# littlemesie/recommend-tf2.0

Hardware: NVIDIA B200
Metric: DLRM train samples/sec (higher is better)
Workload: dtype f32

## Files before the change

### include/rtf_b200.h

```cpp
#ifndef RTF_B200_H
#define RTF_B200_H

#include <stddef.h>
#include <stdint.h>

#ifdef __cplusplus
extern "C" {
#endif

#define RTF_MAX_FIELDS 64

#define RTF_E_ARG (-1)
#define RTF_E_ALIGN (-2)
#define RTF_E_RANGE (-3)
#define RTF_E_WORKSPACE (-4)

enum { RTF_POOL_NONE = 0, RTF_POOL_SUM = 1, RTF_POOL_MEAN = 2,
       RTF_POOL_SKIP_INVALID = 0x100 };
enum { RTF_OPT_NONE = 0, RTF_OPT_SGD = 1, RTF_OPT_ADAGRAD = 2, RTF_OPT_ADAM = 3 };

typedef struct rtf_opt {
  int32_t kind;
  float lr;
  float beta1;
// ... 176 lines not shown
int rtf_layernorm_workspace(int64_t rows, int C, size_t* bytes);
int rtf_layernorm_fwd(const float* d_x, int64_t rows, int C, const float* d_gamma,
                      const float* d_beta, float eps, float* d_y, float* d_mean, float* d_rstd,
                      void* stream);
int rtf_layernorm_bwd(const float* d_dy, const float* d_x, const float* d_mean, const float* d_rstd,
                      const float* d_gamma, int64_t rows, int C, float* d_dx, float* d_dgamma,
                      float* d_dbeta, void* d_ws, size_t ws_bytes, void* stream);

int rtf_dense_gemm_nn_workspace(int M, int N, int K, int batch, size_t* bytes);
int rtf_dense_gemm_nt_workspace(int M, int N, int K, int batch, size_t* bytes);
int rtf_dense_gemm_tn_workspace(int M, int N, int K, int batch, size_t* bytes);
int rtf_dense_gemm_nn(const float* d_a, int64_t lda, int64_t stride_a, const float* d_b, int64_t ldb,
                      int64_t stride_b, const float* d_bias, int relu, float* d_out, int64_t ldd,
                      int64_t stride_d, int M, int N, int K, int batch, void* d_ws, size_t ws_bytes,
                      void* stream);
int rtf_dense_gemm_nt(const float* d_a, int64_t lda, int64_t stride_a, const float* d_b, int64_t ldb,
                      int64_t stride_b, const float* d_bias, int relu, float* d_out, int64_t ldd,
                      int64_t stride_d, int M, int N, int K, int batch, void* d_ws, size_t ws_bytes,
                      void* stream);
int rtf_dense_gemm_tn(const float* d_a, int64_t lda, int64_t stride_a, const float* d_b, int64_t ldb,
                      int64_t stride_b, const float* d_bias, int relu, float* d_out, int64_t ldd,
                      int64_t stride_d, int M, int N, int K, int batch, void* d_ws, size_t ws_bytes,
                      void* stream);

int rtf_autoint_layer_supported(int F, int dm, int H, int hs);
int rtf_autoint_layer_workspace(int64_t B, int dm, int HS, size_t* bytes);
int rtf_autoint_layer_fwd(const float* d_x, int64_t B, int F, int dm, const float* d_wq,
                          const float* d_wk, const float* d_wv, const float* d_w0, int H, int hs,
                          int act, float scale, float* d_out, void* stream);
int rtf_autoint_layer_bwd(const float* d_x, int64_t B, int F, int dm, const float* d_wq,
                          const float* d_wk, const float* d_wv, const float* d_w0, int H, int hs,
                          int act, float scale, const float* d_out, const float* d_gout,
                          float* d_gx, float* d_gw, void* d_ws, size_t ws_bytes, void* stream);

int rtf_sasrec_score_fwd(const float* d_info, int64_t info_sb, const float* d_pos_tab,
                         int64_t pos_rows, const float* d_neg_tab, int64_t neg_rows,
                         const void* d_pos_ids, const void* d_neg_ids, int ids_i64, int64_t neg_sb,
                         int64_t B, int NEG, int D, float* d_logits, float* d_loss_rows,
                         int32_t* d_err, void* stream);
int rtf_sasrec_score_bwd(const float* d_info, int64_t info_sb, const float* d_pos_tab,
                         int64_t pos_rows, const float* d_neg_tab, int64_t neg_rows,
                         const void* d_pos_ids, const void* d_neg_ids, int ids_i64, int64_t neg_sb,
                         int64_t B, int NEG, int D, const float* d_logits, const float* d_gloss,
                         const float* d_glogits, float* d_ginfo, float* d_gemb, void* stream);

int rtf_topk_ip_workspace(int64_t B, int64_t N, int D, int k, size_t* bytes);
// ... 20 lines not shown
```

### recommend-tf2.0_b200/_lib.py

```python
from __future__ import annotations

import ctypes as C
import os
import subprocess
import sys

_HERE = os.path.dirname(os.path.abspath(__file__))
LIB_PATH = os.path.join(_HERE, "librtf_b200.so")
CSRC_DIR = os.path.join(_HERE, "csrc")
HEADER_PATH = os.path.join(os.path.dirname(_HERE), "include", "rtf_b200.h")

POOL_NONE, POOL_SUM, POOL_MEAN = 0, 1, 2
OPT_NONE, OPT_SGD, OPT_ADAGRAD, OPT_ADAM = 0, 1, 2, 3
SEG_CHUNK = 64
MAX_FIELDS = 64


class RtfError(RuntimeError):
    pass


class rtf_opt(C.Structure):
    _fields_ = [("kind", C.c_int32), ("lr", C.c_float), ("beta1", C.c_float),
                ("beta2", C.c_float), ("eps", C.c_float), ("l2", C.c_float),
# ... 50 lines not shown
    "rtf_sasrec_score_bwd": [_p, _i64, _p, _i64, _p, _i64, _p, _p, _int, _i64, _i64, _int, _int, _p, _p, _p,
                             _p, _p, _p],
    "rtf_topk_ip_workspace": [_i64, _i64, _int, _int, C.POINTER(C.c_size_t)],
    "rtf_topk_ip": [_p, _i64, _i64, _p, _i64, _i64, _int, _int, _p, _p, _p, _p, C.c_size_t, _p],
    "rtf_peer_pull_rows": [_p, _p, _i64, _int, C.c_uint64, _p, _int, _int, _p, _int, _i64, _i64, _i64, _p,
                           _i64, _p, _p],
    "rtf_ssm_gather": [_p, _p, _p, _p, _i64, _int, _int, _p, _p, _p, _p],
    "rtf_ssm_logits_fwd": [_p, _i64, _p, _i64, _p, _p, _p, _p, _p, _p, _i64, _i64, _int, _int, _int, _p, _p,
                           _p, _p],
    "rtf_ssm_logits_bwd": [_p, _i64, _p, _i64, _p, _p, _p, _p, _p, _p, _i64, _i64, _int, _int, _int, _p, _p,
                           _p, _p, _i64, _p],
    "rtf_ssm_true_gx": [_p, _p, _p, _i64, _i64, _int, _p, _i64, _p],
    "rtf_dense_adam": [_p, _p, _p, _p, _i64, C.POINTER(rtf_opt), _p],
    "rtf_rows_apply_dense": [_p, _p, _p, _p, _p, _i64, _int, C.POINTER(rtf_opt), _p],
    "rtf_dense_gemm_nn_workspace": [_int, _int, _int, _int, C.POINTER(C.c_size_t)],
    "rtf_dense_gemm_nt_workspace": [_int, _int, _int, _int, C.POINTER(C.c_size_t)],
    "rtf_dense_gemm_tn_workspace": [_int, _int, _int, _int, C.POINTER(C.c_size_t)],
    "rtf_dense_gemm_nn": [_p, _i64, _i64, _p, _i64, _i64, _p, _int, _p, _i64, _i64, _int, _int, _int,
                          _int, _p, C.c_size_t, _p],
    "rtf_dense_gemm_nt": [_p, _i64, _i64, _p, _i64, _i64, _p, _int, _p, _i64, _i64, _int, _int, _int,
                          _int, _p, C.c_size_t, _p],
    "rtf_dense_gemm_tn": [_p, _i64, _i64, _p, _i64, _i64, _p, _int, _p, _i64, _i64, _int, _int, _int,
                          _int, _p, C.c_size_t, _p],
    "rtf_fm_layer_workspace": [_i64, _int, C.POINTER(C.c_size_t)],
    "rtf_fm_layer_fwd": [_p, _i64, _p, _int, _p, _i64, _int, _int, _i64, _int, _int, _p, _p, _p],
    "rtf_fm_layer_bwd": [_p, _i64, _p, _int, _p, _i64, _int, _int, _i64, _int, _int, _p, _p,
                         _i64, _p, _p, _i64, _p, _p],
    "rtf_fm_gather_fwd": [_p, _p, _int, _int, _int, _p, _int, _p, _i64, _p, _int, _i64, _i64,
                          _i64, _p, _p, _p, _p, _p],
    "rtf_fm_gather_bwd": [_p, _p, _int, _int, _int, _p, _int, _p, _i64, _p, _int, _i64, _i64,
                          _i64, _p, _p, _p, _p, _p, _p, _p],
    "rtf_attn_fwd": [_p, _i64, _i64, _p, _i64, _i64, _p, _i64, _i64, _p, _i64, _p, _i64, _int,
                     _int, _int, _int, _int, _int, C.c_float, _p, _i64, _i64, _p, _p, _p],
    "rtf_attn_bwd": [_p, _i64, _i64, _p, _i64, _i64, _p, _i64, _i64, _p, _i64, _p, _i64, _int,
                     _int, _int, _int, _int, _int, C.c_float, _p, _i64, _i64, _p, _p, _p, _i64,
                     _i64, _p, _p, _i64, _i64, _p, _i64, _i64, _p, _i64, _i64, _p],
    "rtf_din_attn_fwd": [_p, _i64, _p, _i64, _p, _i64, _p, _i64, _p, _p, _int, _i64, _int, _int,
                         _p, _i64, _p],
    "rtf_din_attn_bwd": [_p, _i64, _p, _i64, _p, _i64, _p, _i64, _p, _p, _int, _i64, _int, _int,
                         _p, _i64, _p, _i64, _p, _i64, _p, _i64, _p, _p],
    "rtf_log_uniform_workspace": [_int, C.POINTER(C.c_size_t)],
    "rtf_log_uniform_sample": [C.c_uint64, _int, _i64, _p, _p, _p, _p],
    "rtf_log_uniform_sample_dseed": [_p, _int, _i64, _p, _p, _p, _p],
    "rtf_log_uniform_expected": [_p, _i64, _i64, _p, _p, _p],
    "rtf_sampled_softmax_workspace": [_int, _int, C.POINTER(C.c_size_t)],
    "rtf_sampled_softmax_fwd": [_p, _i64, _p, _p, _p, _p, _p, _p, _i64, _i64, _int, _int, _int,
# ... 61 lines not shown
```

### recommend-tf2.0_b200/core.py

```python
from __future__ import annotations

import math
import os
from typing import Callable, Optional, Sequence

import torch
import torch.nn.functional as F


class Layer(torch.nn.Module):

    def __init__(self, name: Optional[str] = None, **kwargs):
        super().__init__()
        self._built = False
        self._name = name

    def build(self, input_shape):
        pass

    def call(self, inputs, **kwargs):
        raise NotImplementedError

    def forward(self, inputs, *args, **kwargs):
        if not self._built:
# ... 76 lines not shown
             lambda x: torch.softmax(x, -1)}
    if act not in table:
        raise ValueError(f"Unknown activation function: {act}")
    return table[act]


class Dense(Layer):

    def __init__(self, units: int, activation=None, use_bias: bool = True,
                 kernel_regularizer=None, **kwargs):
        super().__init__(**kwargs)
        self.units, self.use_bias, self.kernel_regularizer = units, use_bias, kernel_regularizer
        self.activation = get_activation(activation)
        self._act_name = activation if isinstance(activation, str) else None
        if isinstance(activation, torch.nn.Module):
            self.activation_module = activation

    def build(self, input_shape):
        self.kernel = self.add_weight("kernel", (input_shape[-1], self.units), "glorot_uniform",
                                      self.kernel_regularizer)
        self.bias = self.add_weight("bias", (self.units,), "zeros") if self.use_bias else None

    def call(self, x, **kwargs):
        if self.bias is not None and x.dim() >= 2 and x.is_cuda:
            relu = self._act_name == "relu"
            lead = x.shape[:-1]
            x2 = x.reshape(-1, x.shape[-1]) if x.dim() > 2 else x
            y = _DenseFn.apply(x2, self.kernel, self.bias, relu)
            if x.dim() > 2:
                y = y.reshape(*lead, self.units)
            return y if (relu or self.activation is None) else self.activation(y)
        y = torch.matmul(x, self.kernel)
        if self.bias is not None:
            y = y + self.bias
        return self.activation(y) if self.activation is not None else y


DENSE_GEMM = os.environ.get("RTF_DENSE_GEMM", "bf16x6")


def set_dense_gemm(kind: str) -> None:
    global DENSE_GEMM
    if kind not in ("bf16x6", "library"):
        raise ValueError(kind)
    DENSE_GEMM = kind

# ... 2 lines not shown
    if DENSE_GEMM != "bf16x6":
        return False
    for m in mats:
        if not (m.is_cuda and m.dtype == torch.float32 and m.dim() == 2 and m.is_contiguous()
                and m.shape[0] % 4 == 0 and m.shape[1] % 4 == 0 and m.data_ptr() % 16 == 0):
            return False
    return True


def dense_gemm(kind: str, a: torch.Tensor, b: torch.Tensor, bias=None, relu: bool = False,
               splits: int = 1) -> torch.Tensor:
    import ctypes as C
    from . import _lib as L
    lib = L.lib()
    if kind == "nn":
        (M, K), N = a.shape, b.shape[1]
    elif kind == "nt":
        (M, K), N = a.shape, b.shape[0]
    elif kind == "tn":
        (K, M), N = a.shape, b.shape[1]
    else:
        raise ValueError(kind)
    fn = getattr(lib, f"rtf_dense_gemm_{kind}")
    wsq = getattr(lib, f"rtf_dense_gemm_{kind}_workspace")
    lda, ldb = a.stride(0), b.stride(0)
    sa = sb = sd = 0
    batch = 1
    if kind == "tn" and splits > 1:
        if K % splits or (K // splits) % 4:
            raise ValueError("splits must divide K into multiples of 4")
        batch, K = splits, K // splits
        sa, sb, sd = K * lda, K * ldb, M * N
    out = torch.empty((batch, M, N) if batch > 1 else (M, N), dtype=torch.float32, device=a.device)
    key = (kind, M, N, K, batch)
    if key not in _GEMM_WS_BYTES:
        nb = C.c_size_t(0)
        L.check(wsq(M, N, K, batch, C.byref(nb)), f"rtf_dense_gemm_{kind}_workspace")
        _GEMM_WS_BYTES[key] = max(nb.value, 16)
    ws = _scratch(_GEMM_WS_BYTES[key], a.device)
    rc = fn(a.data_ptr(), lda, sa, b.data_ptr(), ldb, sb, None if bias is None else bias.data_ptr(),
            int(relu), out.data_ptr(), N, sd, M, N, K, batch, ws.data_ptr(), ws.numel(),
            L.current_stream_ptr())
    L.check(rc, f"rtf_dense_gemm_{kind}")
    return out.sum(0) if batch > 1 else out


_GEMM_WS_BYTES: dict = {}
_SCRATCH: dict = {}


def _scratch(nbytes: int, device) -> torch.Tensor:
    key = (device.index, torch._C._cuda_getCurrentRawStream(device.index if device.index is not None
                                                            else torch._C._cuda_getDevice()))
    buf = _SCRATCH.get(key)
    if buf is None or buf.numel() < nbytes:
        buf = _SCRATCH[key] = torch.empty(max(nbytes, 1 << 20), dtype=torch.uint8, device=device)
    return buf


def _wgrad_splits(B: int, kin: int, n: int, clusters: int = 74) -> int:
    tiles = ((kin + 255) // 256) * ((n + 127) // 128)
    best, best_eff = 1, 0.0
    s = 1
    while s <= 64 and B % s == 0 and (B // s) % 4 == 0 and B // s >= 512:
        waves = tiles * s / clusters
        eff = waves / -(-tiles * s // clusters)
        if eff > best_eff + 0.02:
# ... 14 lines not shown

def _relu_bwd_bias_grad(gy: torch.Tensor, y):
    B, N = gy.shape
    if gy.is_cuda and N % 4 == 0 and B > 0:
        import ctypes as C
        from . import _lib as L
        gy = gy.contiguous()
        key = ("relu_bwd", B, N)
        if key not in _GEMM_WS_BYTES:
            nb = C.c_size_t(0)
            L.check(L.lib().rtf_relu_bwd_colsum_workspace(B, N, C.byref(nb)), "rtf_relu_bwd_colsum_workspace")
            _GEMM_WS_BYTES[key] = max(nb.value, 16)
        ws = _scratch(_GEMM_WS_BYTES[key], gy.device)
        g = torch.empty_like(gy) if y is not None else gy
        db = torch.empty(N, dtype=torch.float32, device=gy.device)
        L.check(L.lib().rtf_relu_bwd_colsum(gy.data_ptr(), None if y is None else y.data_ptr(), B, N,
                                            g.data_ptr(), db.data_ptr(), ws.data_ptr(),
                                            L.current_stream_ptr()), "rtf_relu_bwd_colsum")
        return g, db
    g = torch.ops.aten.threshold_backward(gy, y, 0.0) if y is not None else gy.contiguous()
    return g, g.sum(0)


class _DenseFn(torch.autograd.Function):

    @staticmethod
    def forward(ctx, x, w, b, relu):
        kpad = 0
        if (x.shape[1] % 4 and DENSE_GEMM == "bf16x6" and x.is_cuda and x.shape[0] >= 1024
                and w.shape[1] % 4 == 0 and x.shape[0] % 4 == 0):
            kpad = (-x.shape[1]) % 4
            x = F.pad(x, (0, kpad))
            w = F.pad(w, (0, 0, 0, kpad))
        ctx.kpad = kpad
        if x.shape[0] >= 1024 and _x6_ok(x, w) and b.data_ptr() % 16 == 0:
            y = dense_gemm("nn", x, w, b, relu)
        else:
            y = torch._addmm_activation(b, x, w, use_gelu=False) if relu else torch.addmm(b, x, w)
        ctx.save_for_backward(x, w, y if relu else None)
        ctx.relu = relu
        return y

    @staticmethod
    def backward(ctx, gy):
        x, w, y = ctx.saved_tensors
        g, gb = _relu_bwd_bias_grad(gy, y if ctx.relu else None)
        gx = None
        if ctx.needs_input_grad[0]:
            gx = dense_gemm("nt", g, w) if (g.shape[0] >= 1024 and _x6_ok(g, w)) else g @ w.t()
        gw = _wgrad(x, g) if ctx.needs_input_grad[1] else None
        if ctx.kpad:
            gx = None if gx is None else gx[:, : gx.shape[1] - ctx.kpad].contiguous()
            gw = None if gw is None else gw[: gw.shape[0] - ctx.kpad]
        return gx, gw, gb, None


class _BatchNormTrainFn(torch.autograd.Function):

    @staticmethod
    def forward(ctx, x2, gamma, beta, eps, momentum, moving_mean, moving_var):
        import ctypes as C
        from . import _lib as L
        L.require_cuda(x2, "BatchNormalization(x)")
        if x2.dtype != torch.float32:
            raise TypeError("BatchNormalization: fp32 activations only")
        if x2.stride(1) != 1:
            x2 = x2.contiguous()
        B, Cc = x2.shape
        key = ("bn", B, Cc)
        if key not in _GEMM_WS_BYTES:
            nb = C.c_size_t(0)
            L.check(L.lib().rtf_bn_workspace(B, Cc, C.byref(nb)), "rtf_bn_workspace")
            _GEMM_WS_BYTES[key] = nb.value
        ws = _scratch(_GEMM_WS_BYTES[key], x2.device)
        y = torch.empty((B, Cc), dtype=torch.float32, device=x2.device)
        stats = torch.empty((2, Cc), dtype=torch.float32, device=x2.device)
        L.check(L.lib().rtf_bn_fwd(x2.data_ptr(), x2.stride(0), B, Cc,
# ... 66 lines not shown

class Dropout(Layer):
    def __init__(self, rate: float = 0.0, **kwargs):
        super().__init__(**kwargs)
        self.rate = rate

    def call(self, x, **kwargs):
        return F.dropout(x, self.rate, self.training) if self.rate > 0 else x


class DNN(Layer):

    def __init__(self, hidden_units: Sequence[int], activation="relu", dnn_dropout: float = 0.0,
                 input_bn: bool = True, **kwargs):
        super().__init__(**kwargs)
        self.dnn_network = torch.nn.ModuleList([Dense(u, activation=activation) for u in hidden_units])
        self.dropout = Dropout(dnn_dropout)
        self.bn = BatchNormalization() if input_bn else None

    def call(self, inputs, **kwargs):
        x = inputs
        if self.bn is not None:
            x = self.bn(x)
        for dnn in self.dnn_network:
            x = dnn(x)
        return self.dropout(x)


class DenseAdam:

    ALIGN = 64

    def __init__(self, params, lr: float = 1e-3, beta1: float = 0.9, beta2: float = 0.999,
                 eps: float = 1e-7):
        from . import _lib as L
        params = [p for p in params if p.requires_grad]
        if not params:
            raise ValueError("DenseAdam: no trainable parameters")
        for p in params:
            L.require_cuda(p, "DenseAdam(param)")
            if p.dtype != torch.float32:
                raise TypeError("DenseAdam: fp32 parameters only")
        self.params, self.lr, self.beta1, self.beta2, self.eps = params, lr, beta1, beta2, eps
        self.t = 0
        self.lr_dev = None
        offs, n = [], 0
        for p in params:
            offs.append(n)
            n += (p.numel() + self.ALIGN - 1) // self.ALIGN * self.ALIGN
# ... 149 lines not shown
```

### recommend-tf2.0_b200/csrc/dense_epilogue.cu

```cuda
#include "rtf_common.cuh"

namespace rtf {

constexpr int RB_ROWS = 128;
constexpr int RB_MAX_CHUNKS = 512;

__global__ void __launch_bounds__(128)
relu_bwd_colsum_stage1(const float* __restrict__ gy, const float* __restrict__ y, long long B,
                       int Ccols, int lx, int rb, float* __restrict__ g, float* __restrict__ partial) {
  const int tx = threadIdx.x % lx, ty = threadIdx.x / lx, ny = 128 / lx;
  const int c4 = (blockIdx.x * lx + tx) * 4;
  if (c4 >= Ccols) return;
  const int sub = rb / ny;
  const long long b0 = (long long)blockIdx.y * rb + (long long)ty * sub;
  const long long b1 = min(b0 + sub, B);
  float4 acc = make_float4(0.f, 0.f, 0.f, 0.f);
  for (long long b = b0; b < b1; ++b) {
    const float4 gv = *reinterpret_cast<const float4*>(gy + b * Ccols + c4);
    float4 o = gv;
    if (y) {
      const float4 yv = *reinterpret_cast<const float4*>(y + b * Ccols + c4);
      o.x = yv.x > 0.f ? gv.x : 0.f;
      o.y = yv.y > 0.f ? gv.y : 0.f;
      o.z = yv.z > 0.f ? gv.z : 0.f;
// ... 14 lines not shown
  const int c = blockIdx.x * 32 + lane;
  float acc = 0.f;
  if (c < Ccols) {
    int k = grp;
    for (; k + (RB2_UNROLL - 1) * RB2_WARPS < nchunks; k += RB2_UNROLL * RB2_WARPS) {
      float a[RB2_UNROLL];
#pragma unroll
      for (int u = 0; u < RB2_UNROLL; ++u) a[u] = partial[(long long)(k + u * RB2_WARPS) * Ccols + c];
#pragma unroll
      for (int u = 0; u < RB2_UNROLL; ++u) acc = __fadd_rn(acc, a[u]);
    }
    for (; k < nchunks; k += RB2_WARPS) acc = __fadd_rn(acc, partial[(long long)k * Ccols + c]);
  }
  part[grp][lane] = acc;
  __syncthreads();
  if (grp == 0 && c < Ccols) {
    float t = part[0][lane];
#pragma unroll
    for (int g = 1; g < RB2_WARPS; ++g) t = __fadd_rn(t, part[g][lane]);
    out[c] = t;
  }
}

}

using namespace rtf;

static int relu_bwd_rb(long long B) {
  const long long per = (long long)RB_ROWS * RB_MAX_CHUNKS;
  return (int)(RB_ROWS * ((B + per - 1) / per > 0 ? (B + per - 1) / per : 1));
}

static int relu_bwd_lx(int cols) {
  const int v = cols / 4;
  return v <= 32 ? 32 : (v <= 64 ? 64 : 128);
}

extern "C" int rtf_relu_bwd_colsum_workspace(int64_t B, int cols, size_t* bytes) {
  if (!bytes || B < 0 || cols <= 0) return RTF_E_ARG;
  const size_t ny = 128 / relu_bwd_lx(cols);
  const int rb = relu_bwd_rb(B);
  *bytes = (size_t)((B + rb - 1) / rb + 1) * ny * (size_t)cols * 4;
  return 0;
}

extern "C" int rtf_relu_bwd_colsum(const float* d_gy, const float* d_y, int64_t B, int cols,
                                   float* d_g, float* d_colsum, void* d_ws, void* stream) {
  if (B < 0 || cols <= 0 || !d_colsum) return RTF_E_ARG;
  cudaStream_t st = (cudaStream_t)stream;
  if (B == 0) return (int)cudaMemsetAsync(d_colsum, 0, (size_t)cols * 4, st);
  if (!d_gy || !d_ws || (d_y && !d_g)) return RTF_E_ARG;
  if (cols % 4 || (uintptr_t)d_gy % 16 || (uintptr_t)d_y % 16 || (uintptr_t)d_g % 16 ||
      (uintptr_t)d_ws % 16)
    return RTF_E_ALIGN;
  const int rb = relu_bwd_rb(B);
  const int nchunks = (int)((B + rb - 1) / rb);
  const int lx = relu_bwd_lx(cols), ny = 128 / lx;
  dim3 g1((cols / 4 + lx - 1) / lx, nchunks);
  relu_bwd_colsum_stage1<<<g1, 128, 0, st>>>(d_gy, d_y, B, cols, lx, rb, d_g, (float*)d_ws);
  relu_bwd_colsum_stage2<<<(cols + 31) / 32, RB2_WARPS * 32, 0, st>>>((const float*)d_ws, nchunks * ny, cols,
                                                           d_colsum);
  RTF_CHECK_LAUNCH();
  return 0;
}
```

### recommend-tf2.0_b200/csrc/dense_gemm.cuh

```cuda
#pragma once
#include <cfloat>
#include <cstdint>
#include <cuda_runtime.h>

#include "cute/tensor.hpp"
#include "cutlass/cutlass.h"
#include "cutlass/epilogue/collective/collective_builder.hpp"
#include "cutlass/epilogue/fusion/operations.hpp"
#include "cutlass/epilogue/thread/activation.h"
#include "cutlass/gemm/collective/collective_builder.hpp"
#include "cutlass/gemm/device/gemm_universal_adapter.h"
#include "cutlass/gemm/kernel/gemm_universal.hpp"
#include "cutlass/numeric_types.h"

#include "rtf_b200.h"

namespace rtf_gemm {

using namespace cute;

using RowMajor = cutlass::layout::RowMajor;
using ColumnMajor = cutlass::layout::ColumnMajor;

template <class LayoutA, class LayoutB, int Bands, class MmaTile = Shape<_256, _128, _32>,
          class Cluster = Shape<_2, _1, _1>,
          class MainSchedule = cutlass::gemm::KernelTmaWarpSpecialized2SmFastFP32SmemSm100,
          class EpiSchedule = cutlass::epilogue::TmaWarpSpecialized2Sm, class ElementC = void,
          int PromotionInterval = 2, class AccCopyAtom = void>
struct FastF32Gemm {
  using Arch = cutlass::arch::Sm100;
  using OpClass = cutlass::arch::OpClassTensorOp;
  using Fusion = cutlass::epilogue::fusion::LinCombPerColBiasEltAct<
      cutlass::epilogue::thread::Clamp, float, float, float, ElementC, float>;
  using Epilogue = typename cutlass::epilogue::collective::CollectiveBuilder<
      Arch, OpClass, MmaTile, Cluster, cutlass::epilogue::collective::EpilogueTileAuto, float,
      float, ElementC, RowMajor, 4, float, RowMajor, 4, EpiSchedule, Fusion>::CollectiveOp;
  using Stock = typename cutlass::gemm::collective::CollectiveBuilder<
      Arch, OpClass, float, LayoutA, 4, float, LayoutB, 4, float, MmaTile, Cluster,
      cutlass::gemm::collective::StageCountAutoCarveout<static_cast<int>(
          sizeof(typename Epilogue::SharedStorage))>,
      MainSchedule>::CollectiveOp;
  using SP = typename Stock::DispatchPolicy;
  using Policy = cutlass::gemm::MainloopSm100TmaUmmaWarpSpecializedFastF32<
      SP::Load2TransformPipelineStageCount, SP::Transform2MmaPipelineStageCount,
      SP::Schedule::SchedulerPipelineStageCount, SP::Schedule::AccumulatorPipelineStageCount, Bands,
      SP::ScalingFactor, (PromotionInterval > 0 ? PromotionInterval : SP::AccPromotionInterval),
      typename SP::ClusterShape,
      cute::conditional_t<cute::is_void_v<AccCopyAtom>, typename SP::AccumulatorCopyAtom, AccCopyAtom>,
      typename SP::ArchTag>;
  using Mainloop = cutlass::gemm::collective::CollectiveMma<
      Policy, typename Stock::TileShape, float, typename Stock::StrideA, float,
      typename Stock::StrideB, typename Stock::TiledMma, typename Stock::GmemTiledCopyA,
      typename Stock::SmemLayoutAtomsA, typename Stock::CopyAtomsA, typename Stock::TransformA,
      typename Stock::GmemTiledCopyB, typename Stock::SmemLayoutAtomsB, typename Stock::CopyAtomsB,
      typename Stock::TransformB>;
  using Kernel = cutlass::gemm::kernel::GemmUniversal<Shape<int, int, int, int>, Mainloop, Epilogue>;
  using Gemm = cutlass::gemm::device::GemmUniversalAdapter<Kernel>;
  using StrideA = typename Kernel::StrideA;
  using StrideB = typename Kernel::StrideB;
  using StrideD = typename Kernel::StrideD;

  template <class Stride, bool KContiguous>
  static Stride make_stride(int64_t ld, int64_t batch) {
    Stride s{};
    if constexpr (KContiguous) {
      get<0>(s) = ld;
    } else {
      get<1>(s) = ld;
    }
    get<2>(s) = batch;
    return s;
  }

  static typename Gemm::Arguments make_args(const float* A, int64_t lda, int64_t sA, const float* B,
                                            int64_t ldb, int64_t sB, const float* bias, float lo,
                                            float hi, float* D, int64_t ldd, int64_t sD, int M, int N,
                                            int K, int batch) {
    constexpr bool a_k = std::is_same_v<LayoutA, RowMajor>;
    constexpr bool b_k = std::is_same_v<LayoutB, ColumnMajor>;
    StrideA sa = make_stride<StrideA, a_k>(lda, sA);
    StrideB sb = make_stride<StrideB, b_k>(ldb, sB);
    StrideD sd = make_stride<StrideD, true>(ldd, sD);
    typename Gemm::Arguments args{cutlass::gemm::GemmUniversalMode::kGemm,
                                  {M, N, K, batch},
                                  {A, sa, B, sb},
                                  {{}, nullptr, sd, D, sd}};
    args.epilogue.thread.alpha = 1.f;
    args.epilogue.thread.beta = 0.f;
    args.epilogue.thread.bias_ptr = bias;
    args.epilogue.thread.activation.lower_bound = lo;
    args.epilogue.thread.activation.upper_bound = hi;
    static int sm_count = 0;
    int dev = 0;
    cudaGetDevice(&dev);
    if (sm_count == 0) cudaDeviceGetAttribute(&sm_count, cudaDevAttrMultiProcessorCount, dev);
    args.hw_info.device_id = dev;
    args.hw_info.sm_count = sm_count;
    return args;
  }

  static int workspace(int M, int N, int K, int batch, size_t* bytes) {
    auto args = make_args(nullptr, K, 0, nullptr, K, 0, nullptr, 0.f, 0.f, nullptr, N, 0, M, N, K, batch);
    *bytes = Gemm::get_workspace_size(args);
    return 0;
  }

  static int run(const float* A, int64_t lda, int64_t sA, const float* B, int64_t ldb, int64_t sB,
                 const float* bias, int relu, float* D, int64_t ldd, int64_t sD, int M, int N, int K,
                 int batch, void* ws, size_t ws_bytes, cudaStream_t st) {
    if (!A || !B || !D || M <= 0 || N <= 0 || K <= 0 || batch <= 0) return RTF_E_ARG;
    if (lda % 4 || ldb % 4 || ldd % 4 || sA % 4 || sB % 4 || sD % 4 || (uintptr_t)A % 16 ||
        (uintptr_t)B % 16 || (uintptr_t)D % 16 || (uintptr_t)bias % 16)
      return RTF_E_ALIGN;
    const float lo = relu ? 0.f : -INFINITY, hi = INFINITY;
    auto args = make_args(A, lda, sA, B, ldb, sB, bias, lo, hi, D, ldd, sD, M, N, K, batch);
    Gemm gemm;
    if (gemm.can_implement(args) != cutlass::Status::kSuccess) return RTF_E_RANGE;
    if (Gemm::get_workspace_size(args) > ws_bytes) return RTF_E_WORKSPACE;
    if (gemm.initialize(args, ws, st) != cutlass::Status::kSuccess) return RTF_E_ARG;
    cutlass::Status s = gemm.run(st);
    if (s != cutlass::Status::kSuccess) return (int)cudaGetLastError() ? (int)cudaGetLastError() : RTF_E_ARG;
    return 0;
  }
};

}
```

### recommend-tf2.0_b200/csrc/dense_gemm_nn.cu

```cuda
#include "dense_gemm.cuh"

using G = rtf_gemm::FastF32Gemm<rtf_gemm::RowMajor, rtf_gemm::RowMajor, RTF_GEMM_BANDS>;

extern "C" int rtf_dense_gemm_nn_workspace(int M, int N, int K, int batch, size_t* bytes) {
  if (!bytes) return RTF_E_ARG;
  return G::workspace(M, N, K, batch, bytes);
}

extern "C" int rtf_dense_gemm_nn(const float* d_a, int64_t lda, int64_t stride_a, const float* d_b,
                                 int64_t ldb, int64_t stride_b, const float* d_bias, int relu,
                                 float* d_out, int64_t ldd, int64_t stride_d, int M, int N, int K,
                                 int batch, void* d_ws, size_t ws_bytes, void* stream) {
  return G::run(d_a, lda, stride_a, d_b, ldb, stride_b, d_bias, relu, d_out, ldd, stride_d, M, N, K,
                batch, d_ws, ws_bytes, (cudaStream_t)stream);
}
```

### recommend-tf2.0_b200/csrc/dense_gemm_nt.cu

```cuda
#include "dense_gemm.cuh"

using G = rtf_gemm::FastF32Gemm<rtf_gemm::RowMajor, rtf_gemm::ColumnMajor, RTF_GEMM_BANDS>;

extern "C" int rtf_dense_gemm_nt_workspace(int M, int N, int K, int batch, size_t* bytes) {
  if (!bytes) return RTF_E_ARG;
  return G::workspace(M, N, K, batch, bytes);
}

extern "C" int rtf_dense_gemm_nt(const float* d_a, int64_t lda, int64_t stride_a, const float* d_b,
                                 int64_t ldb, int64_t stride_b, const float* d_bias, int relu,
                                 float* d_out, int64_t ldd, int64_t stride_d, int M, int N, int K,
                                 int batch, void* d_ws, size_t ws_bytes, void* stream) {
  return G::run(d_a, lda, stride_a, d_b, ldb, stride_b, d_bias, relu, d_out, ldd, stride_d, M, N, K,
                batch, d_ws, ws_bytes, (cudaStream_t)stream);
}
```

### recommend-tf2.0_b200/csrc/rtf_common.cuh

```cuda
#pragma once
#include <cuda_runtime.h>
#include <stdint.h>

#include "rtf_b200.h"

#if defined(__CUDA_ARCH__) && (__CUDA_ARCH__ < 1000)
#error "librtf_b200 is written for sm_100a (B200) only"
#endif

#define RTF_CHECK_LAUNCH()                         \
  do {                                             \
    cudaError_t e__ = cudaGetLastError();          \
    if (e__ != cudaSuccess) return (int)e__;       \
  } while (0)

namespace rtf {

constexpr int kNumSMs = 148;

constexpr float kPadLogit = -4294967296.0f;

__device__ __forceinline__ float4 ldg_nc_f4(const float* p) {
  float4 r;
  asm volatile("ld.global.nc.L1::no_allocate.v4.f32 {%0,%1,%2,%3}, [%4];"
// ... 53 lines not shown
      "r"(parity)
      : "memory");
}
__device__ __forceinline__ void bulk_g2s(void* smem_dst, const void* gmem_src, uint32_t bytes,
                                         uint64_t* bar) {
  asm volatile(
      "cp.async.bulk.shared::cluster.global.mbarrier::complete_tx::bytes [%0], [%1], %2, [%3];" ::
          "r"(smem_u32(smem_dst)),
      "l"(gmem_src), "r"(bytes), "r"(smem_u32(bar))
      : "memory");
}

template <typename IdT>
__device__ __forceinline__ long long load_id(const IdT* ids, long long idx, long long rows,
                                             int32_t* err) {
  long long id = (long long)__ldg(ids + idx);
  if (id < 0 || id >= rows) {
    if (err) atomicOr(err, 1);
    return -1;
  }
  return id;
}

}
```

Baseline: 8.720 million.

## Emit ReLU bitmask in MLP forward GEMM and fuse masking into backward

For all-ReLU DNN stacks, the forward GEMM epilogue now writes a 1-bit ReLU mask alongside the activations. The backward data-gradient GEMM applies the next layer's mask in its epilogue, so the separate relu-backward pass over saved activations is skipped. A custom head kernel for the final 1-unit Dense computes the masked input gradient and bias sum in one pass and hands them to the preceding layer through a link object. The change adds custom CUTLASS epilogue visitors, 2-SM tile configurations and fragile pointer and version matching in autograd, and it only triggers when layer widths are multiples of 128.

Result: faster. 8.961 million, median of 6 (+2.8%).

```diff
diff --git a/include/rtf_b200.h b/include/rtf_b200.h
--- a/include/rtf_b200.h
+++ b/include/rtf_b200.h
@@ -222,6 +222,16 @@
                       int64_t stride_b, const float* d_bias, int relu, float* d_out, int64_t ldd,
                       int64_t stride_d, int M, int N, int K, int batch, void* d_ws, size_t ws_bytes,
                       void* stream);
+int rtf_dense_gemm_nn_relu_bits(const float* d_a, int64_t lda, const float* d_b, int64_t ldb,
+                                const float* d_bias, float* d_out, int64_t ldd, void* d_bits, int M,
+                                int N, int K, void* d_ws, size_t ws_bytes, void* stream);
+int rtf_dense_gemm_nt_mask(const float* d_a, int64_t lda, const float* d_b, int64_t ldb,
+                           const void* d_bits, float* d_out, int64_t ldd, int M, int N, int K,
+                           void* d_ws, size_t ws_bytes, void* stream);
+
+int rtf_dense_head_gx_workspace(int64_t B, int C, size_t* bytes);
+int rtf_dense_head_gx(const float* d_dlogit, const float* d_w, const void* d_bits, int64_t B, int C,
+                      float* d_gx, float* d_db, void* d_ws, void* stream);
 
 int rtf_autoint_layer_supported(int F, int dm, int H, int hs);
 int rtf_autoint_layer_workspace(int64_t B, int dm, int HS, size_t* bytes);
diff --git a/recommend-tf2.0_b200/_lib.py b/recommend-tf2.0_b200/_lib.py
--- a/recommend-tf2.0_b200/_lib.py
+++ b/recommend-tf2.0_b200/_lib.py
@@ -96,6 +96,11 @@
                           _int, _p, C.c_size_t, _p],
     "rtf_dense_gemm_tn": [_p, _i64, _i64, _p, _i64, _i64, _p, _int, _p, _i64, _i64, _int, _int, _int,
                           _int, _p, C.c_size_t, _p],
+    "rtf_dense_gemm_nn_relu_bits": [_p, _i64, _p, _i64, _p, _p, _i64, _p, _int, _int, _int, _p,
+                                    C.c_size_t, _p],
+    "rtf_dense_gemm_nt_mask": [_p, _i64, _p, _i64, _p, _p, _i64, _int, _int, _int, _p, C.c_size_t, _p],
+    "rtf_dense_head_gx_workspace": [_i64, _int, C.POINTER(C.c_size_t)],
+    "rtf_dense_head_gx": [_p, _p, _p, _i64, _int, _p, _p, _p, _p],
     "rtf_fm_layer_workspace": [_i64, _int, C.POINTER(C.c_size_t)],
     "rtf_fm_layer_fwd": [_p, _i64, _p, _int, _p, _i64, _int, _int, _i64, _int, _int, _p, _p, _p],
     "rtf_fm_layer_bwd": [_p, _i64, _p, _int, _p, _i64, _int, _int, _i64, _int, _int, _p, _p,
diff --git a/recommend-tf2.0_b200/core.py b/recommend-tf2.0_b200/core.py
--- a/recommend-tf2.0_b200/core.py
+++ b/recommend-tf2.0_b200/core.py
@@ -122,6 +122,9 @@
         self.bias = self.add_weight("bias", (self.units,), "zeros") if self.use_bias else None
 
     def call(self, x, **kwargs):
+        link = getattr(x, "_rtf_head_link", None)
+        if link is not None and self.units == 1 and self.activation is None and self.bias is not None:
+            return _DenseHeadFn.apply(x, self.kernel, self.bias, link)
         if self.bias is not None and x.dim() >= 2 and x.is_cuda:
             relu = self._act_name == "relu"
             lead = x.shape[:-1]
@@ -170,7 +173,6 @@
     else:
         raise ValueError(kind)
     fn = getattr(lib, f"rtf_dense_gemm_{kind}")
-    wsq = getattr(lib, f"rtf_dense_gemm_{kind}_workspace")
     lda, ldb = a.stride(0), b.stride(0)
     sa = sb = sd = 0
     batch = 1
@@ -180,17 +182,48 @@
         batch, K = splits, K // splits
         sa, sb, sd = K * lda, K * ldb, M * N
     out = torch.empty((batch, M, N) if batch > 1 else (M, N), dtype=torch.float32, device=a.device)
-    key = (kind, M, N, K, batch)
-    if key not in _GEMM_WS_BYTES:
-        nb = C.c_size_t(0)
-        L.check(wsq(M, N, K, batch, C.byref(nb)), f"rtf_dense_gemm_{kind}_workspace")
-        _GEMM_WS_BYTES[key] = max(nb.value, 16)
-    ws = _scratch(_GEMM_WS_BYTES[key], a.device)
+    ws = _gemm_workspace(kind, M, N, K, batch, a.device)
     rc = fn(a.data_ptr(), lda, sa, b.data_ptr(), ldb, sb, None if bias is None else bias.data_ptr(),
             int(relu), out.data_ptr(), N, sd, M, N, K, batch, ws.data_ptr(), ws.numel(),
             L.current_stream_ptr())
     L.check(rc, f"rtf_dense_gemm_{kind}")
     return out.sum(0) if batch > 1 else out
+
+
+def _gemm_workspace(kind: str, M: int, N: int, K: int, batch: int, device) -> torch.Tensor:
+    import ctypes as C
+    from . import _lib as L
+    key = (kind, M, N, K, batch)
+    if key not in _GEMM_WS_BYTES:
+        nb = C.c_size_t(0)
+        wsq = getattr(L.lib(), f"rtf_dense_gemm_{kind}_workspace")
+        L.check(wsq(M, N, K, batch, C.byref(nb)), f"rtf_dense_gemm_{kind}_workspace")
+        _GEMM_WS_BYTES[key] = max(nb.value, 16)
+    return _scratch(_GEMM_WS_BYTES[key], device)
+
+
+def dense_relu_bits(x: torch.Tensor, w: torch.Tensor, b: torch.Tensor):
+    from . import _lib as L
+    (M, K), N = x.shape, w.shape[1]
+    y = torch.empty((M, N), dtype=torch.float32, device=x.device)
+    bits = torch.empty((M, N // 8), dtype=torch.uint8, device=x.device)
+    ws = _gemm_workspace("nn", M, N, K, 1, x.device)
+    L.check(L.lib().rtf_dense_gemm_nn_relu_bits(x.data_ptr(), x.stride(0), w.data_ptr(), w.stride(0),
+                                                b.data_ptr(), y.data_ptr(), N, bits.data_ptr(), M, N, K,
+                                                ws.data_ptr(), ws.numel(), L.current_stream_ptr()),
+            "rtf_dense_gemm_nn_relu_bits")
+    return y, bits
+
+
+def dense_gemm_nt_mask(g: torch.Tensor, w: torch.Tensor, bits: torch.Tensor) -> torch.Tensor:
+    from . import _lib as L
+    (M, K), N = g.shape, w.shape[0]
+    out = torch.empty((M, N), dtype=torch.float32, device=g.device)
+    ws = _gemm_workspace("nt", M, N, K, 1, g.device)
+    L.check(L.lib().rtf_dense_gemm_nt_mask(g.data_ptr(), g.stride(0), w.data_ptr(), w.stride(0),
+                                           bits.data_ptr(), out.data_ptr(), N, M, N, K, ws.data_ptr(),
+                                           ws.numel(), L.current_stream_ptr()), "rtf_dense_gemm_nt_mask")
+    return out
 
 
 _GEMM_WS_BYTES: dict = {}
@@ -251,10 +284,14 @@
     return g, g.sum(0)
 
 
+def _gemm_fwd_ok(x: torch.Tensor, w: torch.Tensor, b: torch.Tensor) -> bool:
+    return x.shape[0] >= 1024 and _x6_ok(x, w) and b.data_ptr() % 16 == 0
+
+
 class _DenseFn(torch.autograd.Function):
 
     @staticmethod
-    def forward(ctx, x, w, b, relu):
+    def forward(ctx, x, w, b, relu, bits_in=None, emit_bits=False, premasked=None):
         kpad = 0
         if (x.shape[1] % 4 and DENSE_GEMM == "bf16x6" and x.is_cuda and x.shape[0] >= 1024
                 and w.shape[1] % 4 == 0 and x.shape[0] % 4 == 0):
@@ -262,26 +299,97 @@
             x = F.pad(x, (0, kpad))
             w = F.pad(w, (0, 0, 0, kpad))
         ctx.kpad = kpad
-        if x.shape[0] >= 1024 and _x6_ok(x, w) and b.data_ptr() % 16 == 0:
+        bits = None
+        if emit_bits and relu and w.shape[1] % 128 == 0 and _gemm_fwd_ok(x, w, b):
+            y, bits = dense_relu_bits(x, w, b)
+        elif _gemm_fwd_ok(x, w, b):
             y = dense_gemm("nn", x, w, b, relu)
         else:
             y = torch._addmm_activation(b, x, w, use_gelu=False) if relu else torch.addmm(b, x, w)
-        ctx.save_for_backward(x, w, y if relu else None)
+        ctx.save_for_backward(x, w, y if relu else None, bits_in)
         ctx.relu = relu
-        return y
-
-    @staticmethod
-    def backward(ctx, gy):
-        x, w, y = ctx.saved_tensors
-        g, gb = _relu_bwd_bias_grad(gy, y if ctx.relu else None)
+        ctx.premasked = premasked if bits is not None else None
+        if not emit_bits:
+            return y
+        if bits is None:
+            bits = torch.empty(0, dtype=torch.uint8, device=y.device)
+        ctx.mark_non_differentiable(bits)
+        return y, bits
+
+    @staticmethod
+    def backward(ctx, gy, *_):
+        x, w, y, bits_in = ctx.saved_tensors
+        pm = ctx.premasked
+        if pm == "next":
+            g, gb = _relu_bwd_bias_grad(gy, None)
+        elif isinstance(pm, _HeadLink) and pm.delivered(gy):
+            g, gb = gy, pm.take_db()
+        else:
+            g, gb = _relu_bwd_bias_grad(gy, y if ctx.relu else None)
         gx = None
         if ctx.needs_input_grad[0]:
-            gx = dense_gemm("nt", g, w) if (g.shape[0] >= 1024 and _x6_ok(g, w)) else g @ w.t()
+            if bits_in is not None and bits_in.numel():
+                gx = dense_gemm_nt_mask(g, w, bits_in)
+            else:
+                gx = dense_gemm("nt", g, w) if (g.shape[0] >= 1024 and _x6_ok(g, w)) else g @ w.t()
         gw = _wgrad(x, g) if ctx.needs_input_grad[1] else None
         if ctx.kpad:
             gx = None if gx is None else gx[:, : gx.shape[1] - ctx.kpad].contiguous()
             gw = None if gw is None else gw[: gw.shape[0] - ctx.kpad]
-        return gx, gw, gb, None
+        return gx, gw, gb, None, None, None, None
+
+
+class _HeadLink:
+
+    def __init__(self, bits):
+        self.bits, self.gx, self.version, self.db = bits, None, None, None
+
+    def deliver(self, gx, db):
+        self.gx, self.version, self.db = gx, gx._version, db
+
+    def delivered(self, gy) -> bool:
+        gx = self.gx
+        return (gx is not None and gy.data_ptr() == gx.data_ptr() and gy.shape == gx.shape
+                and gy.stride() == gx.stride() and gy._version == self.version)
+
+    def take_db(self):
+        db, self.gx, self.db = self.db, None, None
+        return db
+
+
+class _DenseHeadFn(torch.autograd.Function):
+
+    @staticmethod
+    def forward(ctx, x, w, b, link):
+        ctx.save_for_backward(x, w)
+        ctx.link = link
+        return torch.addmm(b, x, w)
+
+    @staticmethod
+    def backward(ctx, gy):
+        import ctypes as C
+        from . import _lib as L
+        x, w = ctx.saved_tensors
+        link = ctx.link
+        g = gy.contiguous()
+        B, Cc = x.shape
+        gx = None
+        if ctx.needs_input_grad[0]:
+            key = ("head_gx", B, Cc)
+            if key not in _GEMM_WS_BYTES:
+                nb = C.c_size_t(0)
+                L.check(L.lib().rtf_dense_head_gx_workspace(B, Cc, C.byref(nb)), "rtf_dense_head_gx_workspace")
+                _GEMM_WS_BYTES[key] = max(nb.value, 16)
+            ws = _scratch(_GEMM_WS_BYTES[key], x.device)
+            wc = w.contiguous()
+            gx = torch.empty((B, Cc), dtype=torch.float32, device=x.device)
+            db = torch.empty(Cc, dtype=torch.float32, device=x.device)
+            L.check(L.lib().rtf_dense_head_gx(g.data_ptr(), wc.data_ptr(), link.bits.data_ptr(), B, Cc,
+                                              gx.data_ptr(), db.data_ptr(), ws.data_ptr(),
+                                              L.current_stream_ptr()), "rtf_dense_head_gx")
+            link.deliver(gx, db)
+        gw = _wgrad(x, g) if ctx.needs_input_grad[1] else None
+        return gx, gw, g.sum(0), None
 
 
 class _BatchNormTrainFn(torch.autograd.Function):
@@ -394,9 +502,43 @@
         x = inputs
         if self.bn is not None:
             x = self.bn(x)
+        if self._relu_chain_ok(x):
+            return self._relu_chain(x)
         for dnn in self.dnn_network:
             x = dnn(x)
         return self.dropout(x)
+
+    def _relu_chain_ok(self, x) -> bool:
+        units = [d.units for d in self.dnn_network]
+        return (DENSE_GEMM == "bf16x6" and torch.is_grad_enabled() and x.is_cuda and x.dim() == 2
+                and x.dtype == torch.float32 and x.shape[0] >= 1024 and x.shape[0] % 4 == 0
+                and self.dropout.rate == 0 and len(units) > 0
+                and all(d._act_name == "relu" and d.use_bias for d in self.dnn_network)
+                and all(u % 4 == 0 for u in units) and any(u % 128 == 0 for u in units))
+
+    def _relu_chain(self, x):
+        layers = list(self.dnn_network)
+        bits = None
+        for i, d in enumerate(layers):
+            if not d._built:
+                d.build(_shape_of(x))
+                d._built = True
+            last = i + 1 == len(layers)
+            x2 = x if x.is_contiguous() else x.contiguous()
+            emit = d.units % 128 == 0
+            link = _HeadLink(None) if (emit and last) else None
+            premasked = link if last else ("next" if emit else None)
+            out = _DenseFn.apply(x2, d.kernel, d.bias, True, bits, emit, premasked)
+            if emit:
+                x, bits = out
+                if bits.numel() == 0:
+                    bits = None
+                elif link is not None:
+                    link.bits = bits
+                    x._rtf_head_link = link
+            else:
+                x, bits = out, None
+        return x
 
 
 class DenseAdam:
diff --git a/recommend-tf2.0_b200/csrc/dense_epilogue.cu b/recommend-tf2.0_b200/csrc/dense_epilogue.cu
--- a/recommend-tf2.0_b200/csrc/dense_epilogue.cu
+++ b/recommend-tf2.0_b200/csrc/dense_epilogue.cu
@@ -60,19 +60,24 @@
   }
 }
 
-}
-
-using namespace rtf;
-
-static int relu_bwd_rb(long long B) {
+int relu_bwd_rb(long long B) {
   const long long per = (long long)RB_ROWS * RB_MAX_CHUNKS;
   return (int)(RB_ROWS * ((B + per - 1) / per > 0 ? (B + per - 1) / per : 1));
 }
 
-static int relu_bwd_lx(int cols) {
+int relu_bwd_lx(int cols) {
   const int v = cols / 4;
   return v <= 32 ? 32 : (v <= 64 ? 64 : 128);
 }
+
+void relu_bwd_colsum_stage2_launch(const float* partial, int nrows, int cols, float* out,
+                                   cudaStream_t st) {
+  relu_bwd_colsum_stage2<<<(cols + 31) / 32, RB2_WARPS * 32, 0, st>>>(partial, nrows, cols, out);
+}
+
+}
+
+using namespace rtf;
 
 extern "C" int rtf_relu_bwd_colsum_workspace(int64_t B, int cols, size_t* bytes) {
   if (!bytes || B < 0 || cols <= 0) return RTF_E_ARG;
@@ -96,8 +101,7 @@
   const int lx = relu_bwd_lx(cols), ny = 128 / lx;
   dim3 g1((cols / 4 + lx - 1) / lx, nchunks);
   relu_bwd_colsum_stage1<<<g1, 128, 0, st>>>(d_gy, d_y, B, cols, lx, rb, d_g, (float*)d_ws);
-  relu_bwd_colsum_stage2<<<(cols + 31) / 32, RB2_WARPS * 32, 0, st>>>((const float*)d_ws, nchunks * ny, cols,
-                                                           d_colsum);
+  relu_bwd_colsum_stage2_launch((const float*)d_ws, nchunks * ny, cols, d_colsum, st);
   RTF_CHECK_LAUNCH();
   return 0;
 }
diff --git a/recommend-tf2.0_b200/csrc/dense_gemm.cuh b/recommend-tf2.0_b200/csrc/dense_gemm.cuh
--- a/recommend-tf2.0_b200/csrc/dense_gemm.cuh
+++ b/recommend-tf2.0_b200/csrc/dense_gemm.cuh
@@ -22,16 +22,147 @@
 using RowMajor = cutlass::layout::RowMajor;
 using ColumnMajor = cutlass::layout::ColumnMajor;
 
+template <class T>
+struct ReluBit : cutlass::epilogue::thread::Clamp<T> {};
+
+}
+
+namespace cutlass::epilogue::fusion {
+
+template <class ElementOutput, class ElementCompute, FloatRoundStyle RoundStyle, int Stages,
+          class EpilogueTile, class StrideMNL, class SmemLayoutAtom, class CopyOpR2S, int Alignment,
+          bool EnableNullptr, class InputOp>
+struct Sm90TreeVisitor<
+    Sm90Compute<rtf_gemm::ReluBit, ElementOutput, ElementCompute, RoundStyle>,
+    Sm90TreeVisitor<Sm90AuxStore<Stages, EpilogueTile, cutlass::uint1b_t, RoundStyle, StrideMNL,
+                                 SmemLayoutAtom, CopyOpR2S, Alignment, EnableNullptr>,
+                    InputOp>>
+    : Sm90VisitorImpl<Sm90VisitorImpl<InputOp, detail::Sm90ReLUAuxStore<StrideMNL>>,
+                      Sm90Compute<rtf_gemm::ReluBit, ElementOutput, ElementCompute, RoundStyle>> {
+  static_assert(cute::is_same_v<ElementCompute, float>);
+  using Impl = Sm90VisitorImpl<Sm90VisitorImpl<InputOp, detail::Sm90ReLUAuxStore<StrideMNL>>,
+                               Sm90Compute<rtf_gemm::ReluBit, ElementOutput, ElementCompute, RoundStyle>>;
+  using Params = typename Impl::Params;
+  using SharedStorage = typename Impl::SharedStorage;
+
+  CUTLASS_HOST_DEVICE
+  Sm90TreeVisitor() {}
+
+  CUTLASS_HOST_DEVICE
+  Sm90TreeVisitor(Params const& params_, SharedStorage const& shared_storage)
+      : params(params_), Impl(params_, shared_storage) {}
+
+  Params const& params;
+
+  template <class RTensor, class GTensor, class CTensor, class ThrResidue, class CallbacksImpl>
+  struct ConsumerStoreCallbacks : CallbacksImpl {
+    CUTLASS_DEVICE
+    ConsumerStoreCallbacks(RTensor&& tC_rAux, GTensor&& tC_gAux, CTensor tC_cAux,
+                           ThrResidue residue_tC_cAux, Params const& params, CallbacksImpl&& impl)
+        : tC_rAux(cute::forward<RTensor>(tC_rAux)),
+          tC_gAux(cute::forward<GTensor>(tC_gAux)),
+          tC_cAux(tC_cAux),
+          residue_tC_cAux(residue_tC_cAux),
+          params(params),
+          CallbacksImpl(cute::forward<CallbacksImpl>(impl)) {}
+
+    RTensor tC_rAux;
+    GTensor tC_gAux;
+    CTensor tC_cAux;
+    ThrResidue residue_tC_cAux;
+    Params const& params;
+
+    template <typename ElementAccumulator, int FragmentSize>
+    CUTLASS_DEVICE Array<ElementOutput, FragmentSize> visit(
+        Array<ElementAccumulator, FragmentSize> const& frg_acc, int epi_v, int epi_m, int epi_n) {
+      auto& [callbacks_input_aux, callbacks_compute] = CallbacksImpl::callbacks_tuple;
+      auto& [callbacks_input, callbacks_aux] = callbacks_input_aux.callbacks_tuple;
+      auto const& [params_input_aux, params_compute] = params;
+
+      Array frg_input = callbacks_input.visit(frg_acc, epi_v, epi_m, epi_n);
+      using ElementInput = typename decltype(frg_input)::Element;
+      NumericArrayConverter<ElementCompute, ElementInput, FragmentSize, RoundStyle> convert_input{};
+      NumericArrayConverter<ElementOutput, ElementCompute, FragmentSize, RoundStyle> convert_output{};
+      PackPredicates<FragmentSize> convert_aux{};
+      rtf_gemm::ReluBit<ElementCompute> relu{};
+
+      Array frg_compute = convert_input(frg_input);
+      bool frg_aux[FragmentSize];
+      CUTLASS_PRAGMA_UNROLL
+      for (int i = 0; i < FragmentSize; ++i) {
+        frg_compute[i] = relu(frg_compute[i], params_compute);
+        frg_aux[i] = frg_compute[i] > ElementCompute(0);
+      }
+      static_assert(FragmentSize % 8 == 0, "Predicate vector must be byte-aligned");
+      Tensor tC_rAux_frg =
+          recast<typename PackPredicates<FragmentSize>::result_type>(coalesce(tC_rAux));
+      tC_rAux_frg(epi_v) = convert_aux(frg_aux);
+      return convert_output(frg_compute);
+    }
+
+    CUTLASS_DEVICE void end_loop(int epi_m, int epi_n) {
+      CallbacksImpl::end_loop(epi_m, epi_n);
+      Tensor tC_gAux_mn = tC_gAux(_, _, _, epi_m, epi_n);
+      Tensor tC_cAux_mn = tC_cAux(_, _, _, epi_m, epi_n);
+      constexpr auto MCL = decltype(max_common_layout(tC_rAux, tC_gAux_mn)){};
+      constexpr int V = cute::min(Alignment, size(MCL));
+      static_assert(V > 1 && V % 8 == 0, "bit stores must be byte-aligned vectors");
+      using VecType = uint_bit_t<V>;
+      Tensor tC_rAux_vec = recast<VecType>(tC_rAux);
+      Tensor tC_gAux_vec = recast<VecType>(tC_gAux_mn);
+      Tensor tC_cAux_vec = tensor<1>(zipped_divide(tC_cAux_mn, MCL.compose(Int<V>{})));
+      Tensor tC_pAux_vec = cute::lazy::transform(
+          tC_cAux_vec, [&](auto const& c) { return elem_less(c, residue_tC_cAux); });
+      copy_if(tC_pAux_vec, tC_rAux_vec, tC_gAux_vec);
+    }
+  };
+
+  template <bool ReferenceSrc, class... Args>
+  CUTLASS_DEVICE auto get_consumer_store_callbacks(ConsumerStoreArgs<Args...> const& args) {
+    auto const& [params_input_aux, params_compute] = params;
+    auto const& [params_input, params_aux] = params_input_aux;
+
+    auto [M, N, K, L] = args.problem_shape_mnkl;
+    auto [m, n, k, l] = args.tile_coord_mnkl;
+    gmem_ptr ptr_aux = make_gmem_ptr<cutlass::uint1b_t>(params_aux.ptr_aux);
+    Tensor mAux = make_tensor(ptr_aux, make_layout(make_shape(M, N, L), params_aux.dAux));
+    Tensor gAux = local_tile(mAux, take<0, 2>(args.tile_shape_mnk), make_coord(m, n, l));
+    Tensor tC_gAux = sm90_partition_for_epilogue<ReferenceSrc>(gAux, args.epi_tile, args.tiled_copy,
+                                                               args.thread_idx);
+    Tensor tC_rAux = make_tensor<cutlass::uint1b_t>(take<0, 3>(shape(tC_gAux)));
+
+    auto callbacks_impl = Impl::template get_consumer_store_callbacks<ReferenceSrc>(args);
+    return ConsumerStoreCallbacks<decltype(tC_rAux), decltype(tC_gAux), decltype(args.tCcD),
+                                  decltype(args.residue_tCcD), decltype(callbacks_impl)>(
+        cute::move(tC_rAux), cute::move(tC_gAux), args.tCcD, args.residue_tCcD, params,
+        cute::move(callbacks_impl));
+  }
+};
+
+}
+
+namespace rtf_gemm {
+
+template <class ElementC>
+using BiasClamp = cutlass::epilogue::fusion::LinCombPerColBiasEltAct<
+    cutlass::epilogue::thread::Clamp, float, float, float, ElementC, float>;
+using BiasReluBits = cutlass::epilogue::fusion::LinCombPerColBiasEltActAux<
+    RowMajor, ReluBit, float, float, cutlass::uint1b_t, float, void, float>;
+using MaskBits = cutlass::epilogue::fusion::LinCombDeEltAct<
+    RowMajor, cutlass::epilogue::thread::dReLU, float, float, cutlass::uint1b_t, void, float>;
+constexpr int kBitAlign = 128;
+
 template <class LayoutA, class LayoutB, int Bands, class MmaTile = Shape<_256, _128, _32>,
           class Cluster = Shape<_2, _1, _1>,
           class MainSchedule = cutlass::gemm::KernelTmaWarpSpecialized2SmFastFP32SmemSm100,
           class EpiSchedule = cutlass::epilogue::TmaWarpSpecialized2Sm, class ElementC = void,
-          int PromotionInterval = 2, class AccCopyAtom = void>
+          int PromotionInterval = 2, class AccCopyAtom = void, class FusionOp = void>
 struct FastF32Gemm {
   using Arch = cutlass::arch::Sm100;
   using OpClass = cutlass::arch::OpClassTensorOp;
-  using Fusion = cutlass::epilogue::fusion::LinCombPerColBiasEltAct<
-      cutlass::epilogue::thread::Clamp, float, float, float, ElementC, float>;
+  using Fusion = cute::conditional_t<cute::is_void_v<FusionOp>, BiasClamp<ElementC>, FusionOp>;
+  static constexpr bool kBits = !std::is_same_v<Fusion, BiasClamp<ElementC>>;
+  static constexpr bool kMask = std::is_same_v<Fusion, MaskBits>;
   using Epilogue = typename cutlass::epilogue::collective::CollectiveBuilder<
       Arch, OpClass, MmaTile, Cluster, cutlass::epilogue::collective::EpilogueTileAuto, float,
       float, ElementC, RowMajor, 4, float, RowMajor, 4, EpiSchedule, Fusion>::CollectiveOp;
@@ -75,7 +206,7 @@
   static typename Gemm::Arguments make_args(const float* A, int64_t lda, int64_t sA, const float* B,
                                             int64_t ldb, int64_t sB, const float* bias, float lo,
                                             float hi, float* D, int64_t ldd, int64_t sD, int M, int N,
-                                            int K, int batch) {
+                                            int K, int batch, void* bits = nullptr) {
     constexpr bool a_k = std::is_same_v<LayoutA, RowMajor>;
     constexpr bool b_k = std::is_same_v<LayoutB, ColumnMajor>;
     StrideA sa = make_stride<StrideA, a_k>(lda, sA);
@@ -87,9 +218,15 @@
                                   {{}, nullptr, sd, D, sd}};
     args.epilogue.thread.alpha = 1.f;
     args.epilogue.thread.beta = 0.f;
-    args.epilogue.thread.bias_ptr = bias;
-    args.epilogue.thread.activation.lower_bound = lo;
-    args.epilogue.thread.activation.upper_bound = hi;
+    if constexpr (!kMask) {
+      args.epilogue.thread.bias_ptr = bias;
+      args.epilogue.thread.activation.lower_bound = lo;
+      args.epilogue.thread.activation.upper_bound = hi;
+    }
+    if constexpr (kBits) {
+      args.epilogue.thread.aux_ptr = static_cast<cutlass::uint1b_t*>(bits);
+      args.epilogue.thread.dAux = {int64_t(N), _1{}, int64_t(M) * N};
+    }
     static int sm_count = 0;
     int dev = 0;
     cudaGetDevice(&dev);
@@ -107,13 +244,17 @@
 
   static int run(const float* A, int64_t lda, int64_t sA, const float* B, int64_t ldb, int64_t sB,
                  const float* bias, int relu, float* D, int64_t ldd, int64_t sD, int M, int N, int K,
-                 int batch, void* ws, size_t ws_bytes, cudaStream_t st) {
+                 int batch, void* ws, size_t ws_bytes, cudaStream_t st, void* bits = nullptr) {
     if (!A || !B || !D || M <= 0 || N <= 0 || K <= 0 || batch <= 0) return RTF_E_ARG;
     if (lda % 4 || ldb % 4 || ldd % 4 || sA % 4 || sB % 4 || sD % 4 || (uintptr_t)A % 16 ||
         (uintptr_t)B % 16 || (uintptr_t)D % 16 || (uintptr_t)bias % 16)
       return RTF_E_ALIGN;
+    if constexpr (kBits) {
+      if (!bits || (kMask ? bias != nullptr : !relu)) return RTF_E_ARG;
+      if (N % kBitAlign || (uintptr_t)bits % 16) return RTF_E_ALIGN;
+    }
     const float lo = relu ? 0.f : -INFINITY, hi = INFINITY;
-    auto args = make_args(A, lda, sA, B, ldb, sB, bias, lo, hi, D, ldd, sD, M, N, K, batch);
+    auto args = make_args(A, lda, sA, B, ldb, sB, bias, lo, hi, D, ldd, sD, M, N, K, batch, bits);
     Gemm gemm;
     if (gemm.can_implement(args) != cutlass::Status::kSuccess) return RTF_E_RANGE;
     if (Gemm::get_workspace_size(args) > ws_bytes) return RTF_E_WORKSPACE;
diff --git a/recommend-tf2.0_b200/csrc/dense_gemm_nn.cu b/recommend-tf2.0_b200/csrc/dense_gemm_nn.cu
--- a/recommend-tf2.0_b200/csrc/dense_gemm_nn.cu
+++ b/recommend-tf2.0_b200/csrc/dense_gemm_nn.cu
@@ -1,6 +1,12 @@
 #include "dense_gemm.cuh"
 
 using G = rtf_gemm::FastF32Gemm<rtf_gemm::RowMajor, rtf_gemm::RowMajor, RTF_GEMM_BANDS>;
+using GBits = rtf_gemm::FastF32Gemm<rtf_gemm::RowMajor, rtf_gemm::RowMajor, RTF_GEMM_BANDS,
+                                    cute::Shape<cute::_256, cute::_128, cute::_32>,
+                                    cute::Shape<cute::_2, cute::_1, cute::_1>,
+                                    cutlass::gemm::KernelTmaWarpSpecialized2SmFastFP32SmemSm100,
+                                    cutlass::epilogue::TmaWarpSpecialized2Sm, void, 2, void,
+                                    rtf_gemm::BiasReluBits>;
 
 extern "C" int rtf_dense_gemm_nn_workspace(int M, int N, int K, int batch, size_t* bytes) {
   if (!bytes) return RTF_E_ARG;
@@ -14,3 +20,11 @@
   return G::run(d_a, lda, stride_a, d_b, ldb, stride_b, d_bias, relu, d_out, ldd, stride_d, M, N, K,
                 batch, d_ws, ws_bytes, (cudaStream_t)stream);
 }
+
+extern "C" int rtf_dense_gemm_nn_relu_bits(const float* d_a, int64_t lda, const float* d_b, int64_t ldb,
+                                           const float* d_bias, float* d_out, int64_t ldd, void* d_bits,
+                                           int M, int N, int K, void* d_ws, size_t ws_bytes,
+                                           void* stream) {
+  return GBits::run(d_a, lda, 0, d_b, ldb, 0, d_bias, 1, d_out, ldd, 0, M, N, K, 1, d_ws, ws_bytes,
+                    (cudaStream_t)stream, d_bits);
+}
diff --git a/recommend-tf2.0_b200/csrc/dense_gemm_nt.cu b/recommend-tf2.0_b200/csrc/dense_gemm_nt.cu
--- a/recommend-tf2.0_b200/csrc/dense_gemm_nt.cu
+++ b/recommend-tf2.0_b200/csrc/dense_gemm_nt.cu
@@ -1,6 +1,12 @@
 #include "dense_gemm.cuh"
 
 using G = rtf_gemm::FastF32Gemm<rtf_gemm::RowMajor, rtf_gemm::ColumnMajor, RTF_GEMM_BANDS>;
+using GMask = rtf_gemm::FastF32Gemm<rtf_gemm::RowMajor, rtf_gemm::ColumnMajor, RTF_GEMM_BANDS,
+                                    cute::Shape<cute::_256, cute::_128, cute::_32>,
+                                    cute::Shape<cute::_2, cute::_1, cute::_1>,
+                                    cutlass::gemm::KernelTmaWarpSpecialized2SmFastFP32SmemSm100,
+                                    cutlass::epilogue::TmaWarpSpecialized2Sm, void, 2, void,
+                                    rtf_gemm::MaskBits>;
 
 extern "C" int rtf_dense_gemm_nt_workspace(int M, int N, int K, int batch, size_t* bytes) {
   if (!bytes) return RTF_E_ARG;
@@ -14,3 +20,10 @@
   return G::run(d_a, lda, stride_a, d_b, ldb, stride_b, d_bias, relu, d_out, ldd, stride_d, M, N, K,
                 batch, d_ws, ws_bytes, (cudaStream_t)stream);
 }
+
+extern "C" int rtf_dense_gemm_nt_mask(const float* d_a, int64_t lda, const float* d_b, int64_t ldb,
+                                      const void* d_bits, float* d_out, int64_t ldd, int M, int N, int K,
+                                      void* d_ws, size_t ws_bytes, void* stream) {
+  return GMask::run(d_a, lda, 0, d_b, ldb, 0, nullptr, 0, d_out, ldd, 0, M, N, K, 1, d_ws, ws_bytes,
+                    (cudaStream_t)stream, const_cast<void*>(d_bits));
+}
diff --git a/recommend-tf2.0_b200/csrc/dense_head.cu b/recommend-tf2.0_b200/csrc/dense_head.cu
--- /dev/null
+++ b/recommend-tf2.0_b200/csrc/dense_head.cu
@@ -0,0 +1,52 @@
+#include "rtf_common.cuh"
+
+namespace rtf {
+
+__global__ void __launch_bounds__(128)
+dense_head_gx_stage1(const float* __restrict__ dlogit, const float* __restrict__ w,
+                     const uint8_t* __restrict__ bits, long long B, int C, int lx, int rb,
+                     float* __restrict__ gx, float* __restrict__ partial) {
+  const int tx = threadIdx.x % lx, ty = threadIdx.x / lx, ny = 128 / lx;
+  const int c4 = (blockIdx.x * lx + tx) * 4;
+  if (c4 >= C) return;
+  const int sub = rb / ny;
+  const long long b0 = (long long)blockIdx.y * rb + (long long)ty * sub;
+  const long long b1 = min(b0 + sub, B);
+  const float4 wv = *reinterpret_cast<const float4*>(w + c4);
+  float4 acc = make_float4(0.f, 0.f, 0.f, 0.f);
+  for (long long b = b0; b < b1; ++b) {
+    const float d = dlogit[b];
+    const unsigned m = (unsigned)bits[(b * C + c4) >> 3] >> (c4 & 7);
+    const float4 g = make_float4((m & 1u) ? __fmul_rn(d, wv.x) : 0.f, (m & 2u) ? __fmul_rn(d, wv.y) : 0.f,
+                                 (m & 4u) ? __fmul_rn(d, wv.z) : 0.f, (m & 8u) ? __fmul_rn(d, wv.w) : 0.f);
+    *reinterpret_cast<float4*>(gx + b * C + c4) = g;
+    acc = f4_add(acc, g);
+  }
+  *reinterpret_cast<float4*>(partial + ((long long)blockIdx.y * ny + ty) * C + c4) = acc;
+}
+
+}
+
+using namespace rtf;
+
+extern "C" int rtf_dense_head_gx_workspace(int64_t B, int C, size_t* bytes) {
+  return rtf_relu_bwd_colsum_workspace(B, C, bytes);
+}
+
+extern "C" int rtf_dense_head_gx(const float* d_dlogit, const float* d_w, const void* d_bits, int64_t B,
+                                 int C, float* d_gx, float* d_db, void* d_ws, void* stream) {
+  if (B < 0 || C <= 0 || !d_w || !d_db) return RTF_E_ARG;
+  cudaStream_t st = (cudaStream_t)stream;
+  if (B == 0) return (int)cudaMemsetAsync(d_db, 0, (size_t)C * 4, st);
+  if (!d_dlogit || !d_bits || !d_gx || !d_ws) return RTF_E_ARG;
+  if (C % 8 || (uintptr_t)d_w % 16 || (uintptr_t)d_gx % 16 || (uintptr_t)d_ws % 16) return RTF_E_ALIGN;
+  const int rb = relu_bwd_rb(B);
+  const int nchunks = (int)((B + rb - 1) / rb);
+  const int lx = relu_bwd_lx(C), ny = 128 / lx;
+  dim3 g1((C / 4 + lx - 1) / lx, nchunks);
+  dense_head_gx_stage1<<<g1, 128, 0, st>>>(d_dlogit, d_w, (const uint8_t*)d_bits, B, C, lx, rb, d_gx,
+                                           (float*)d_ws);
+  relu_bwd_colsum_stage2_launch((const float*)d_ws, nchunks * ny, C, d_db, st);
+  RTF_CHECK_LAUNCH();
+  return 0;
+}
diff --git a/recommend-tf2.0_b200/csrc/rtf_common.cuh b/recommend-tf2.0_b200/csrc/rtf_common.cuh
--- a/recommend-tf2.0_b200/csrc/rtf_common.cuh
+++ b/recommend-tf2.0_b200/csrc/rtf_common.cuh
@@ -99,4 +99,9 @@
   return id;
 }
 
+int relu_bwd_rb(long long B);
+int relu_bwd_lx(int cols);
+void relu_bwd_colsum_stage2_launch(const float* partial, int nrows, int cols, float* out,
+                                   cudaStream_t st);
+
 }
```
